# MPI-SWS/RedQueen

Measured on AMD Instinct MI355X. Metric: redqueen_replicas_per_sec, higher is better.
Workload: dtype f64; 1 GPU; C3 syn1k: 1000 followers, 50 sources (25 Poisson2 rate 1 + 25 Hawkes l0=1 a=1 b=10), degree 5, T=100, q=1e6, s=1, RedQueen, randomized worlds; replicas_per_gpu=10000, global_batch=10000, parallelism=replica-sharded dp1, replicas_per_chunk=10000

## Files before the change

redqueen_amd/csrc/rq_api.cpp:

```cpp
#include <hip/hip_runtime.h>

#include <algorithm>
#include <cstring>
#include <memory>
#include <mutex>
#include <new>
#include <vector>

#include "../../include/rq.h"
#include "rq_internal.h"

using rqh::align_up;
using rqh::CtrlTables;
using rqh::GraphTopo;
using rqh::Knobs;
using rqh::Plan;

namespace {

template <class T>
struct DevBuf {
    T* p = nullptr;
    size_t n = 0;
    ~DevBuf() { if (p) (void)hipFree(p); }
// ... 102 lines not shown
        lru->caller = caller;
        lru->used = ++clock;
        return *lru;
    }
};
thread_local SidePipes t_pipes;

}

namespace {
constexpr int kStages = 4;
struct Stage {
    void* buf = nullptr;
    size_t bytes = 0;
    hipEvent_t done = nullptr;
};
}

struct rq_graph : GraphTopo {
    DevBuf<int64_t> d_sink_ids, d_src_id;
    DevBuf<int> d_csr_col_el, d_lay_ptr, d_lay_end;
    DevBuf<int> d_tile_ptr, d_tile_col;
    DevBuf<uint32_t> d_mask, d_fbits;
    DevBuf<int> d_kind, d_orig, d_arr_off, d_arr_n, d_csr_ptr, d_csr_col, d_outdeg_f, d_fol, d_cbf;
    DevBuf<uint32_t> d_seed;
    DevBuf<double> d_p0, d_p1, d_p2, d_arr_a, d_arr_b;
    int upload();
    std::mutex stage_mu;
    Stage stage[kStages];
    int stage_next = 0;
    ~rq_graph()
    {
        for (Stage& st : stage) {
            if (st.done) {
                (void)hipEventSynchronize(st.done);
                (void)hipEventDestroy(st.done);
            }
            if (st.buf) (void)hipHostFree(st.buf);
        }
    }
};

int rq_graph::upload()
{
    int rc;
    if (nw > 0 && (rc = d_mask.upload(masks))) return rc;
    if ((rc = d_fbits.upload(fbits))) return rc;
    if ((rc = d_src_id.upload(src_id)) || (rc = d_kind.upload(kind)) ||
        (rc = d_orig.upload(orig_idx)) || (rc = d_arr_off.upload(arr_off)) ||
        (rc = d_arr_n.upload(arr_n)) || (rc = d_csr_ptr.upload(csr_ptr)) ||
        (rc = d_csr_col.upload(csr_col)) || (rc = d_outdeg_f.upload(outdeg_f)) ||
        (rc = d_fol.upload(fol)) || (rc = d_seed.upload(seed)) ||
        (rc = d_p0.upload(p0)) || (rc = d_p1.upload(p1)) ||
        (rc = d_p2.upload(p2)) || (rc = d_arr_a.upload(arr_a)) ||
        (rc = d_arr_b.upload(arr_b)) || (rc = d_sink_ids.upload(sink_ids)) ||
        (rc = d_csr_col_el.upload(csr_col_el)) || (rc = d_cbf.upload(cbf)))
        return rc;
    if (multi && ((rc = d_lay_ptr.upload(lay_ptr)) || (rc = d_lay_end.upload(lay_end))))
        return rc;
    if (n_tiles > 0 && ((rc = d_tile_ptr.upload(tile_ptr)) || (rc = d_tile_col.upload(tile_col))))
        return rc;
    return RQ_OK;
}

namespace {

double ws_budget(const rq_batch_desc* b, const Knobs& kn, double fallback)
{
    double bud = b && b->ws_budget > 0 ? (double)b->ws_budget : fallback;
    if (!(bud > 0.0)) {
        size_t fr = 0, tot = 0;
        bud = hipMemGetInfo(&fr, &tot) == hipSuccess ? 0.9 * (double)fr : 200.0 * (1 << 30);
    }
    if (kn.ws_budget_gb.set) bud = std::min(bud, kn.ws_budget_gb.v * (1 << 30));
    return bud;
}

int plan_call(const rq_graph* g, const rq_batch_desc* b, const Knobs& kn, double fallback, Plan* p)
{
// ... 64 lines not shown
        return rc;
    }
    ~Join() { (void)done(); }
};
int fork_streams(int nbuf, Join* join)
{
    if (nbuf <= 1) return RQ_OK;
    if (const int rc = join->sp.get(nbuf - 1, join->pst + 1)) return rc;
    if (hipEventRecord(join->sp.fork, join->pst[0]) != hipSuccess) return RQ_EHIP;
    for (int k = 1; k < nbuf; ++k) {
        if (hipStreamWaitEvent(join->pst[k], join->sp.fork, 0) != hipSuccess) return RQ_EHIP;
        join->n = k + 1;
    }
    return RQ_OK;
}

struct Chunk {
    int64_t c0, C;
    char* ws;
    char* wsb;
};

GenArgs gen_args(const rq_graph* g, const Plan& p, const rq_batch_desc* b, const rq_outputs* out,
                 const Chunk& ch)
{
    GenArgs ga{};
    ga.n_chunk = ch.C;
    ga.chunk0 = ch.c0;
    ga.rep0 = b->replica0;
    ga.n_rep = b->n_rep;
    ga.rep_lo = p.rep_lo;
    ga.rep_cnt = p.rep_cnt;
    ga.rep_idx = b->rep_idx ? (const int64_t*)(ch.ws + p.off_repidx) : nullptr;
    ga.n_str = g->n_str;
    ga.ctrl_idx = g->ctrl_idx;
    ga.ctrl_stream_kind =
        (b->ctrl_kind == RQ_SRC_OPT || b->ctrl_kind == RQ_SRC_OPTPW || b->ctrl_kind == RQ_SRC_NONE)
            ? RQ_SRC_NONE : b->ctrl_kind;
    ga.randomize = b->randomize_world;
    ga.seed_mod = b->seed_mod;
    ga.ctrl_seed = b->ctrl_seed;
    ga.ctrl_seed0 = b->ctrl_seed0;
    ga.world_seed = b->world_seed;
    ga.world_seed0 = b->world_seed0;
    ga.ctrl_rate = b->ctrl_rate;
    ga.kind = g->d_kind.p;
    ga.orig_idx = g->d_orig.p;
    ga.seed = g->d_seed.p;
    ga.p0 = g->d_p0.p;
    ga.p1 = g->d_p1.p;
    ga.p2 = g->d_p2.p;
    ga.arr_off = g->d_arr_off.p;
    ga.arr_n = g->d_arr_n.p;
    ga.arr_a = g->d_arr_a.p;
    ga.arr_b = g->d_arr_b.p;
    ga.st_off = (const int64_t*)(ch.ws + p.off_stoff);
    ga.cap = (const int*)(ch.ws + p.off_cap);
    ga.capsum = p.capsum;
    ga.start = g->start;
    ga.end = g->end;
    ga.streams = (double*)(ch.wsb + p.off_streams);
    ga.slen = (int*)(ch.wsb + p.off_slen);
    ga.slen_stride = p.chunk;
    ga.status = out->status;
    if (b->n_rd > 0) {
        ga.rd_k = (const int*)(ch.ws + p.off_rdk);
        ga.n_rd = b->n_rd;
        ga.rd_times = b->rd_times;
        ga.rd_off = b->rd_off;
    }
    return ga;
}

MergeArgs merge_args(const rq_graph* g, const Plan& p, const rq_outputs* out, const Chunk& ch,
                     const GenArgs& ga, const Knobs& kn)
{
    MergeArgs ma{};
    ma.n_chunk = ch.C;
    ma.chunk0 = ch.c0;
    ma.n_str = g->n_str;
    ma.capsum = p.capsum;
    ma.st_off = ga.st_off;
    ma.streams = ga.streams;
    ma.slen = ga.slen;
    ma.slen_stride = ga.slen_stride;
    ma.end = g->end;
    ma.out_t = (double*)(ch.wsb + p.off_mt);
    ma.out_j = (uint16_t*)(ch.wsb + p.off_mj);
    ma.out_jh = g->n_str > 65535 ? (uint8_t*)(ch.wsb + p.off_mjh) : nullptr;
    ma.out_len = (int*)(ch.wsb + p.off_mlen);
    ma.mrg_stride = p.mrg_stride;
    ma.status = out->status;
    ma.strict_ties = p.lmrg ? 1 : 0;
// ... 263 lines not shown
                 size_t workspace_bytes, void* hip_stream)
{
    const Knobs kn = rqh::read_knobs();
    Plan p;
    int rc = plan_call(g, b, kn, (double)workspace_bytes, &p);
    if (rc) return rc;
    if (!out || !out->metrics || !out->counts || !out->status || !workspace) return RQ_EINVAL;
    if (workspace_bytes < p.total) return RQ_EINVAL;
    if ((b->flags & RQ_RUN_EVENT_LOG) && (!out->ev_t || !out->ev_src || out->ev_cap < 1))
        return RQ_EINVAL;
    char* ws = (char*)workspace;
    hipStream_t pst[3] = {(hipStream_t)hip_stream, nullptr, nullptr};

    if ((rc = stage_tables(g, p, b, rqh::ctrl_tables(*g, b), ws, pst[0]))) return rc;
    if (hipMemsetAsync(out->status, 0, sizeof(int32_t) * p.R, pst[0]) != hipSuccess) return RQ_EHIP;
    Join join{pst, t_pipes.of(pst[0])};
    if ((rc = fork_streams(p.nbuf, &join))) return rc;

    int64_t ci = 0;
    for (int64_t c0 = 0; c0 < p.R; c0 += p.chunk, ++ci) {
        hipStream_t s = pst[ci % p.nbuf];
        const Chunk ch{c0, std::min(p.chunk, p.R - c0), ws,
                       ws + p.off_set0 + (size_t)(ci % p.nbuf) * p.set_stride};
        const GenArgs ga = gen_args(g, p, b, out, ch);
        if (!p.fw || p.fwm) {
            TimedLaunch tl(K_GEN, s);
            if (rq_launch_gen(ga, s) != hipSuccess) return RQ_EHIP;
        }
        if (p.mrg && (rc = launch_merge(p, merge_args(g, p, out, ch, ga, kn), ch, s))) return rc;
        const SweepArgs sa = sweep_args(g, p, b, out, ch, ga, kn);
        if (p.order && rq_launch_order(sa.mrg_len, ch.C, (int*)(ch.wsb + p.off_ord), s) != hipSuccess)
            return RQ_EHIP;
        if (hipMemsetAsync(ch.wsb + p.off_wq, 0, 2 * sizeof(int), s) != hipSuccess) return RQ_EHIP;
        {
            TimedLaunch tl(K_SWEEP, s);
            const SweepInst inst = rqh::sweep_inst(p, b->ctrl_kind);
            const hipError_t e = inst.fused ? rq_launch_sweep_fw(sa, inst, s) : rq_launch_sweep(sa, inst, s);
            if (e != hipSuccess) return RQ_EHIP;
        }
        if (p.scan) continue;
        const ScanArgs sc = scan_args(g, p, out, ch, sa);
        TimedLaunch tl(K_SCAN, s);
        if (rq_launch_scan(sc, p.nK, s) != hipSuccess) return RQ_EHIP;
    }
    return join.done();
}

// ... 707 lines not shown
```

redqueen_amd/csrc/rq_gen.h:

```cpp
#pragma once
#include "rq_device.h"
#include "rq_internal.h"

namespace rq {

struct SrcGen {
    uint32_t k0, k1;
    uint32_t d;
    double en, e1n, u2n;
    int kind;
    bool done;
    double t;
    double tau, eta, B;
    double inv;
    double p0, p1, nbeta;
    const uint64_t* etab;
    const double* ta;
    const double* tb;
    int na, ri;

    __device__ __forceinline__ void none()
    {
        etab = nullptr;
        kind = RQ_SRC_NONE;
        done = true;
        d = 0u;
        en = e1n = u2n = 0.0;
    }
    __device__ __forceinline__ void draw2(uint32_t call, double& e, double& u) const
    {
        uint32_t c[4] = {call, 0u, 0u, 0u};
        philox4x32_10(c, k0, k1);
        e = rq_std_exponential(rq_uniform53(c[0], c[1]));
        u = rq_uniform53(c[2], c[3]);
    }

    __device__ __forceinline__ void init(const GenArgs& a, int j, int64_t i, const uint64_t* etab_)
    {
        etab = etab_;
        const bool is_ctrl = j == a.ctrl_idx;
        kind = is_ctrl ? a.ctrl_stream_kind : a.kind[j];
        const int64_t k = a.seed_mod > 0 ? i % a.seed_mod : i;
        uint32_t seed;
        if (is_ctrl) {
            seed = a.ctrl_seed ? a.ctrl_seed[i] : a.ctrl_seed0 + (uint32_t)k;
        } else if (a.randomize) {
            const uint32_t u = a.world_seed ? a.world_seed[i] : a.world_seed0 + (uint32_t)k;
            seed = u + 99u * (uint32_t)a.orig_idx[j];
        } else {
            seed = a.seed[j];
        }
        k0 = seed;
        k1 = kind_salt(kind, is_ctrl);
        d = 0u;
        en = e1n = u2n = 0.0;
        done = false;
        t = a.start;
        tau = a.start;
        eta = 0.0;
        B = 0.0;
        inv = 0.0;
        p0 = p1 = nbeta = 0.0;
        ta = tb = nullptr;
        na = ri = 0;
        if (kind == RQ_SRC_POISSON || kind == RQ_SRC_POISSON2) {
            const double rate = is_ctrl ? a.ctrl_rate[i] : a.p0[j];
            if (rate > 0.0) inv = 1.0 / rate;
            else done = true;
        } else if (kind == RQ_SRC_HAWKES) {
            p0 = a.p0[j];
            p1 = a.p1[j];
            nbeta = -a.p2[j];
            B = p0;
            if (B > 0.0) inv = 1.0 / B;
            else done = true;
        } else if (kind == RQ_SRC_PWCONST) {
            na = a.arr_n[j];
            ta = a.arr_a + a.arr_off[j];
            tb = a.arr_b + a.arr_off[j];
            double mx = tb[0];
            for (int q = 1; q < na; ++q) mx = tb[q] > mx ? tb[q] : mx;
            if (mx > 0.0) inv = 1.0 / mx;
            else done = true;
            p0 = mx;
        } else if (kind == RQ_SRC_REALDATA) {
            const int rk = (a.rd_k && !is_ctrl) ? a.rd_k[j] : -1;
            if (rk >= 0) {
                const int64_t o = a.rd_off[i * a.n_rd + rk];
                na = (int)(a.rd_off[i * a.n_rd + rk + 1] - o);
                ta = a.rd_times + o;
            } else {
                na = a.arr_n[j];
                ta = a.arr_a + a.arr_off[j];
            }
            done = na <= 0;
        } else {
            done = true;
        }
        if (!done && (kind == RQ_SRC_HAWKES || kind == RQ_SRC_PWCONST)) draw2(0u, e1n, u2n);
    }

    __device__ __forceinline__ bool step(double* out, double end)
    {
        if (done) return false;
        if (kind == RQ_SRC_REALDATA) {
            *out = ta[ri];
            ++ri;
            done = ri >= na;
            return true;
        }
        const bool poisson = kind == RQ_SRC_POISSON || kind == RQ_SRC_POISSON2;
        double e, u2 = 0.0;
        if (poisson) {
            if ((d & 1u) == 0u) {
                uint32_t c[4] = {d >> 1, 0u, 0u, 0u};
                philox4x32_10(c, k0, k1);
                e = rq_std_exponential(rq_uniform53(c[0], c[1]));
                en = rq_std_exponential(rq_uniform53(c[2], c[3]));
            } else {
                e = en;
            }
            d += 1u;
        } else {
            e = e1n;
            u2 = u2n;
            d += 2u;
            draw2(d >> 1, e1n, u2n);
        }
        const double tc = t + e * inv;
        if (!(tc <= end)) {
            done = true;
            return false;
        }
        t = tc;
        if (poisson) {
            *out = tc;
            return true;
        }
        if (kind == RQ_SRC_HAWKES) {
            const double decay = rq_exp_t(nbeta * (tc - tau), etab);
            const double rate = p0 + eta * decay;
            const bool acc = u2 * B < rate;
            if (acc) {
                eta = eta * decay + p1;
                tau = tc;
                B = p0 + eta;
            } else {
                B = rate;
            }
            if (B > 0.0) inv = 1.0 / B;
            else done = true;
            if (acc) *out = tc;
            return acc;
        }
        int lo = 0, hi = na;
        while (lo < hi) {
            const int mid = (lo + hi) >> 1;
            if (tc < ta[mid]) hi = mid;
            else lo = mid + 1;
        }
        int idx = lo - 1;
        if (idx < 0) idx += na;
        if (u2 * p0 < tb[idx]) {
            *out = tc;
            return true;
        }
        return false;
    }
};

}
```

redqueen_amd/csrc/rq_host.h:

```cpp
#pragma once
#include <stddef.h>
#include <stdint.h>

#include <vector>

#include "../../include/rq.h"

#define RQ_MAX_STREAMS 2048
#define RQ_NPSUM1_LDS 516
#ifndef RQ_MRG_LB
#define RQ_MRG_LB 1024
#endif
#define RQ_MG_B 512
#define RQ_MAX_STREAMS_MRG (RQ_MG_B * RQ_MG_B)

struct SweepInst {
    bool fused;
    int nK;
    bool col16;
    bool log;
    bool gs;
    bool bits;
    bool bl;
    bool mrg;
// ... 28 lines not shown

inline int followers_tiles(int n_sinks) { return (n_sinks + RQ_FOLLOWERS_TILE_SINKS - 1) / RQ_FOLLOWERS_TILE_SINKS; }
inline size_t followers_tiled_ws_bytes(int n_sinks, int64_t n_rep)
{
    return align_up((size_t)4 * (size_t)n_rep * (size_t)followers_tiles(n_sinks), 256);
}

template <class T>
struct Knob {
    bool set = false;
    T v{};
};
struct Knobs {
    Knob<double> ws_budget_gb;
    double cap_squeeze = 1.0;
    Knob<int> mg_grp;
    bool mrg = true;
    Knob<int> g_collds;
    int g_w = 0;
    bool skip = true;
    bool fwm = true;
    bool ctrl_draws = true;
    bool sweep_scan = true;
    bool phasec_blk = true;
    int fw_w = 0;
    int pipe = 2;
    Knob<int64_t> pipe_chunk;
    bool order = false;

    int sweep_dbg = 0;
    double fw_tile = 58.0;
    Knob<int> fw_hmin, fw_thr, fw_hfill;
    int fw_static = 0;
    bool clk_merge = false;

    Knob<int> rp_chunk;
    bool rp_small = true;
    bool clk_replay = false;

    int lm_of_slots = 4096;
};
Knobs read_knobs();

struct GraphTopo {
    int n_str = 0, ctrl_idx = -1, n_sinks = 0, n_fol = 0;
    int64_t n_edges = 0, ctrl_src_id = 0;
    double start = 0.0, end = 0.0;
    std::vector<int64_t> src_id;
    std::vector<int> kind, orig_idx, arr_off, arr_n;
    std::vector<int> is_static;
    std::vector<uint32_t> seed;
    std::vector<double> p0, p1, p2, arr_a, arr_b;
    std::vector<int> csr_ptr, csr_col, outdeg_f, fol;
    std::vector<int64_t> fol_ids;
    std::vector<int64_t> sink_ids;
    std::vector<int> csr_col_el;
    std::vector<int> col_to_fol;
    bool multi = false, ctrl_dup = false;
    bool rd_ties = false, rd_ties_ctrl = false;
    std::vector<int> lay_ptr, lay_end;
    int nw = 0;
    std::vector<uint32_t> masks;
    std::vector<uint32_t> fbits;
    std::vector<int> cbf;
    int n_tiles = 0;
    std::vector<int> tile_ptr, tile_col;
    int ctrl_arr_off = 0, ctrl_arr_n = 0;
};
int topo_build(const rq_graph_desc* d, GraphTopo* g);

struct Plan {
    int nK = 1, spl = 1, wpb = 4, n_sinks_pad = 0;
    int64_t R = 0, chunk = 0, capsum = 0, cap_rows = 0;
    int64_t rep_lo = 0, rep_cnt = 0;
    std::vector<int> cap;
    std::vector<int64_t> st_off;
    std::vector<int> rd_k;
    bool log = false, bits = false;
    bool bl = false;
    size_t g_fb = 0, g_etab = 0, g_inv = 0, g_skip = 0;
    bool g_inv_sh = false;
    bool gs = false;
    int64_t gs_slots = 0, gs_stride = 0;
    bool fw = false;
    int fw_h = 8, mstride = 1;
    bool mrg = false;
    bool lmrg = false;
// ... 68 lines not shown
```

redqueen_amd/csrc/rq_internal.h:

```cpp
#pragma once
#include <hip/hip_runtime.h>
#include <stdint.h>

#include <map>
#include <mutex>
#include <tuple>

#include "../../include/rq.h"
#include "rq_host.h"
#include "rq_log_walk.h"

__host__ __device__ __forceinline__ int64_t rq_global_replica(int64_t s, int64_t n_rep, int64_t rep_lo,
                                                               int64_t rep_cnt)
{
    return rep_cnt == n_rep ? s : (s / rep_cnt) * n_rep + rep_lo + s % rep_cnt;
}

struct GenArgs {
    int64_t n_chunk, chunk0, rep0;
    int64_t n_rep, rep_lo, rep_cnt;
    const int64_t* rep_idx;
    int n_str, ctrl_idx, ctrl_stream_kind, randomize;
    int64_t seed_mod;
    const uint32_t* ctrl_seed;
    uint32_t ctrl_seed0;
    const uint32_t* world_seed;
    uint32_t world_seed0;
    const double* ctrl_rate;
    const int* kind;
    const int* orig_idx;
    const uint32_t* seed;
    const double *p0, *p1, *p2;
    const int *arr_off, *arr_n;
    const double *arr_a, *arr_b;
    const int64_t* st_off;
    const int* cap;
    int64_t capsum;
    double start, end;
    double* streams;
    int* slen;
    int64_t slen_stride;
    int32_t* status;
    const int* rd_k;
    int n_rd;
    const double* rd_times;
    const int64_t* rd_off;
};

__host__ __device__ __forceinline__ int64_t rq_replica_of(const GenArgs& a, int64_t local)
{
    return a.rep_idx ? a.rep_idx[local] : rq_global_replica(a.rep0 + local, a.n_rep, a.rep_lo, a.rep_cnt);
}

struct SweepArgs {
    int64_t n_chunk, chunk0, n_rep, rep0;
    int wpb, n_str, n_sinks, n_sinks_pad, ctrl_idx, ctrl_kind, n_fol;
    int Ks[RQ_MAX_K];
    int64_t ctrl_src_id;
    int64_t seed_mod;
    const uint32_t* ctrl_seed;
    uint32_t ctrl_seed0;
    const int64_t* src_id;
    const double* inv_c;
    const double* pw_c;
    const double* pw_max;
    int n_seg;
    double period;
    const int* csr_ptr;
    const int* csr_col;
// ... 387 lines not shown
```

redqueen_amd/csrc/rq_kernels.hip:

```cpp
#include <hip/hip_runtime.h>
#include <stdint.h>

#include "rq_device.h"
#include "rq_internal.h"
#include "rq_sweep_core.h"
#include "rq_gen.h"
#include "rq_scan_rows.h"
#include <type_traits>
#include <algorithm>
#include <cstdlib>

#pragma clang fp contract(off)

using namespace rq;

__global__ __launch_bounds__(256) void rq_gen_streams(GenArgs a)
{
    __shared__ uint64_t etab[RQ_EXP_TAB_N];
    for (int e = threadIdx.x; e < RQ_EXP_TAB_N; e += blockDim.x) etab[e] = rq_exp_tab_c[e];
    __syncthreads();
    const int64_t rl = (int64_t)blockIdx.x * blockDim.x + threadIdx.x;
    const int j = (int)(blockIdx.z * gridDim.y + blockIdx.y);
    if (rl >= a.n_chunk || j >= a.n_str) return;
    const int64_t o = a.chunk0 + rl;
    const int64_t i = rq_replica_of(a, o);
    SrcGen gen;
    gen.init(a, j, i, etab);

    double* out = a.streams + rl * a.capsum + a.st_off[j];
    const int cap = a.cap[j];
    int n = 0;
    bool ovf = false;
#ifndef RQ_GEN_W
#define RQ_GEN_W 16
#endif
    constexpr int GW = RQ_GEN_W;
    static_assert(GW == 8 || GW == 16, "staging width");
    double sb[GW];
#pragma unroll
    for (int k = 0; k < GW; ++k) sb[k] = 0.0;
    while (!gen.done && !ovf) {
        double tv;
        if (gen.step(&tv, a.end)) {
            if (n < cap) {
#pragma unroll
                for (int k = 0; k + 1 < GW; ++k) sb[k] = sb[k + 1];
                sb[GW - 1] = tv;
                ++n;
                if ((n & (GW - 1)) == 0) {
                    double4* d = reinterpret_cast<double4*>(out + n - GW);
#pragma unroll
                    for (int k = 0; k < GW / 4; ++k) d[k] = make_double4(sb[4 * k], sb[4 * k + 1], sb[4 * k + 2], sb[4 * k + 3]);
                }
            } else {
                ovf = true;
            }
        }
    }
    {
        const int r = n & (GW - 1);
        if (r > 0) {
#ifndef RQ_GEN_TAIL_STEPS
#define RQ_GEN_TAIL_STEPS 1
#endif
            const int sh = GW - r;
#pragma unroll
            for (int st = 1; st < GW; st <<= 1) {
                const bool on = (sh & st) != 0;
#pragma unroll
                for (int k = 0; k < GW; ++k) {
#if RQ_GEN_TAIL_STEPS
                    const double up = sb[k + st < GW ? k + st : GW - 1], keep = sb[k];
                    sb[k] = on ? up : keep;
#else
                    sb[k] = on ? sb[k + st < GW ? k + st : GW - 1] : sb[k];
#endif
                }
            }
            double4* d = reinterpret_cast<double4*>(out + (n - r));
#pragma unroll
            for (int k = 0; k < GW / 4; ++k)
                if (k < 2 || r > 8) d[k] = make_double4(sb[4 * k], sb[4 * k + 1], sb[4 * k + 2], sb[4 * k + 3]);
        }
    }
    a.slen[(int64_t)j * a.slen_stride + rl] = n;
    if (ovf) atomicOr(&a.status[o], RQ_ST_STREAM_OVERFLOW);
}

template <int SPL, int NK, class COL, int W, bool LOG, bool BITS, bool BL, bool GS = false, bool MRG = false,
          bool GT = false>
__global__ __launch_bounds__(LOG ? 256 : (MRG ? RQ_MRG_LB : (SPL >= 4 ? 512 : 1024))) void rq_sweep(SweepArgs a)
{
    extern __shared__ double lds_g[];
    char* base = reinterpret_cast<char*>(lds_g);
    const int lane = lane_id();
    const int w = __builtin_amdgcn_readfirstlane((int)(threadIdx.x >> 6));
    int* cptr = reinterpret_cast<int*>(base + a.lds_ptr);
    int* odf = reinterpret_cast<int*>(base + a.lds_odf);
    int* cbf = reinterpret_cast<int*>(base + a.lds_cbf);
    constexpr bool col_lds = sizeof(COL) == 2;
    COL* col_l = reinterpret_cast<COL*>(base + a.lds_col);
    const int* col_g = a.csr_col;
    if (col_lds && !BITS)
        for (int e = threadIdx.x; e < a.n_csr; e += blockDim.x) col_l[e] = (COL)a.csr_col[e];
    uint32_t* msk = reinterpret_cast<uint32_t*>(base + a.lds_mask);
    if (BITS)
        for (int e = threadIdx.x; e < a.n_str * a.mstride; e += blockDim.x) {
            const int jj = e / a.mstride, ww = e - jj * a.mstride;
            msk[e] = ww < a.nw ? a.masks[jj * a.nw + ww] : 0u;
        }
// ... 908 lines not shown
}

static int occ_t(SweepKernel k, int wpb, size_t lds)
{
    return rq_occupancy(k, 64 * wpb, lds);
}
static hipError_t launch_sweep_t(SweepKernel k, bool gs, const SweepArgs& a, hipStream_t s)
{
    unsigned blocks = (unsigned)((a.n_chunk + a.wpb - 1) / a.wpb);
    if (a.wq) {
        const int nb_c = occ_t(k, a.wpb, a.lds_total);
        const unsigned cap = (unsigned)(nb_c > 0 ? nb_c : 1) * (unsigned)rq_cu_count();
        if (cap < blocks) blocks = cap;
    }
    if (gs) {
        const unsigned cap = (unsigned)(a.gs_slots / a.wpb);
        if (!a.wq || cap < 1) return hipErrorInvalidValue;
        if (cap < blocks) blocks = cap;
    }
    hipLaunchKernelGGL(k, dim3(blocks), dim3(64 * a.wpb), a.lds_total, s, a);
    return hipGetLastError();
}

hipError_t rq_launch_gen(const GenArgs& a, hipStream_t s)
{
    if (a.n_chunk <= 0 || a.n_str <= 0) return hipSuccess;
    const unsigned gy = (unsigned)std::min(a.n_str, 32768);
    dim3 grid((unsigned)((a.n_chunk + 255) / 256), gy, (unsigned)((a.n_str + gy - 1) / gy));
    hipLaunchKernelGGL(rq_gen_streams, grid, dim3(256), 0, s, a);
    return hipGetLastError();
}

hipError_t rq_launch_sweep(const SweepArgs& a, const SweepInst& i, hipStream_t s)
{
    if (a.n_chunk <= 0) return hipSuccess;
    const SweepKernel k = sweep_kernel(i);
    return k ? launch_sweep_t(k, i.log && i.gs, a, s) : hipErrorInvalidValue;
}

int rq_sweep_blocks_per_cu(const SweepInst& i, int wpb, size_t lds)
{
    const SweepKernel k = sweep_kernel(i);
    return k ? occ_t(k, wpb, lds) : 0;
}

template <int NK>
static hipError_t launch_scan_t(const ScanArgs& a, hipStream_t s)
{
    const size_t lds = 4 * npsum_lds_doubles<NK + 2>() * sizeof(double);
    constexpr auto k = rq_scan<NK, 2>;
    unsigned blocks = (unsigned)((a.n_chunk + 3) / 4);
    if (a.wq) {
        const int nb = rq_occupancy(k, 256, lds);
        const unsigned cap = (unsigned)(nb > 0 ? nb : 1) * (unsigned)rq_cu_count();
        if (cap < blocks) blocks = cap;
// ... 16 lines not shown
```

redqueen_amd/csrc/rq_plan.cpp:

```cpp
#include <algorithm>
#include <cmath>
#include <cstdlib>

#include "rq_host.h"
#include "rq_tables.h"

namespace rqh {

Knobs read_knobs()
{
    Knobs k;
    if (const char* e = getenv("RQ_WS_BUDGET_GB")) k.ws_budget_gb = {true, atof(e)};
    if (const char* e = getenv("RQ_CAP_SQUEEZE")) k.cap_squeeze = std::max(0.01, std::min(1.0, atof(e)));
    if (const char* e = getenv("RQ_MG_GRP")) k.mg_grp = {true, atoi(e)};
    if (const char* e = getenv("RQ_MRG")) k.mrg = atoi(e) != 0;
    if (const char* e = getenv("RQ_G_COLLDS")) k.g_collds = {true, atoi(e)};
    if (const char* e = getenv("RQ_G_W")) k.g_w = atoi(e);
    if (const char* e = getenv("RQ_SKIP")) k.skip = atoi(e) != 0;
    if (const char* e = getenv("RQ_FWM")) k.fwm = atoi(e) != 0;
    if (const char* e = getenv("RQ_CTRL_DRAWS")) k.ctrl_draws = atoi(e) != 0;
    if (const char* e = getenv("RQ_SWEEP_SCAN")) k.sweep_scan = atoi(e) != 0;
    if (const char* e = getenv("RQ_PHASEC_BLK")) k.phasec_blk = atoi(e) != 0;
    if (const char* e = getenv("RQ_FW_W")) k.fw_w = atoi(e);
    if (const char* e = getenv("RQ_PIPE")) k.pipe = std::max(1, std::min(3, atoi(e)));
    if (const char* e = getenv("RQ_PIPE_CHUNK")) k.pipe_chunk = {true, std::max<int64_t>(64, atoll(e))};
    if (const char* e = getenv("RQ_ORDER")) k.order = atoi(e) != 0;
    if (const char* e = getenv("RQ_SWEEP_DBG")) k.sweep_dbg = atoi(e);
    if (const char* e = getenv("RQ_FW_TILE")) k.fw_tile = atof(e);
    if (const char* e = getenv("RQ_FW_HMIN")) k.fw_hmin = {true, atoi(e)};
    if (const char* e = getenv("RQ_FW_THR")) k.fw_thr = {true, atoi(e)};
    if (const char* e = getenv("RQ_FW_HFILL")) k.fw_hfill = {true, atoi(e)};
    static const int fw_static = getenv("RQ_FW_STATIC") ? atoi(getenv("RQ_FW_STATIC")) : 0;
    k.fw_static = fw_static;
    k.clk_merge = getenv("RQ_CLK_MERGE") != nullptr;
    if (const char* e = getenv("RQ_RP_CHUNK")) k.rp_chunk = {true, atoi(e)};
    if (const char* e = getenv("RQ_RP_SMALL")) k.rp_small = atoi(e) != 0;
    k.clk_replay = getenv("RQ_CLK_REPLAY") != nullptr;
    if (const char* e = getenv("RQ_LM_OF_SLOTS")) k.lm_of_slots = std::max(1, std::min(4096, atoi(e)));
    return k;
}

namespace {

constexpr size_t kLdsMax = 160 * 1024;
// ... 484 lines not shown
```

redqueen_amd/csrc/rq_spec.h:

```cpp
#ifndef RQ_SPEC_H
#define RQ_SPEC_H

#include <stdint.h>
#include <math.h>
#include "rq_tables.h"

#if defined(__HIPCC__)
#define RQ_HD __host__ __device__ __forceinline__
#define RQ_HD_COLD static __host__ __device__ __attribute__((noinline))
#pragma clang fp contract(off)
#else
#define RQ_HD static inline
#define RQ_HD_COLD static
#endif

RQ_HD uint64_t rq_dbl_bits(double x)
{
    union { double d; uint64_t u; } c;
    c.d = x;
    return c.u;
}

RQ_HD double rq_bits_dbl(uint64_t u)
{
    union { double d; uint64_t u; } c;
    c.u = u;
    return c.d;
}

RQ_HD double rq_uniform53(uint32_t a, uint32_t b)
{
    return ((double)(a >> 5) * 67108864.0 + (double)(b >> 6)) / 9007199254740992.0;
}

RQ_HD double rq_log(double x)
{
    const double ln2_hi = 6.93147180369123816490e-01;
    const double ln2_lo = 1.90821492927058770002e-10;
    const double Lg1 = 6.666666666666735130e-01;
    const double Lg2 = 3.999999999940941908e-01;
    const double Lg3 = 2.857142874366239149e-01;
    const double Lg4 = 2.222219843214978396e-01;
    const double Lg5 = 1.818357216161805012e-01;
    const double Lg6 = 1.531383769920937332e-01;
    const double Lg7 = 1.479819860511658591e-01;

    uint64_t ux = rq_dbl_bits(x);
    if (!(x > 0.0)) {
        if (x == 0.0) return rq_bits_dbl(0xfff0000000000000ull);
        return rq_bits_dbl(0x7ff8000000000000ull);
    }
    if ((ux >> 52) >= 0x7ffu) return x + x;

    int32_t k = 0;
    if ((ux >> 52) == 0) {
        x = x * 18014398509481984.0;
        ux = rq_dbl_bits(x);
        k = -54;
    }
    int32_t hx = (int32_t)(ux >> 32);
    k += (hx >> 20) - 1023;
    hx &= 0x000fffff;
    int32_t i = (hx + 0x95f64) & 0x100000;
    uint64_t um = ((uint64_t)(uint32_t)(hx | (i ^ 0x3ff00000)) << 32) | (ux & 0xffffffffu);
    k += (i >> 20);
    double f = rq_bits_dbl(um) - 1.0;
    double dk = (double)k;

    double s = f / (2.0 + f);
    double z = s * s;
    double w = z * z;
    double t1 = w * (Lg2 + w * (Lg4 + w * Lg6));
    double t2 = z * (Lg1 + w * (Lg3 + w * (Lg5 + w * Lg7)));
    double R = t2 + t1;
    double hfsq = 0.5 * f * f;
    if (f == 0.0) return dk * ln2_hi + dk * ln2_lo;
    return dk * ln2_hi - ((hfsq - (s * (hfsq + R) + dk * ln2_lo)) - f);
}

RQ_HD double rq_exp_core(double x, const uint64_t* tab, uint64_t adj)
{
    const double kd0 = x * RQ_EXP_INVLN2N + 0x1.8p52;
    const uint64_t ki = rq_dbl_bits(kd0);
    const double kd = kd0 - 0x1.8p52;
    double r = fma(kd, -RQ_EXP_LN2HI, x);
    r = fma(kd, -RQ_EXP_LN2LO, r);
    const uint32_t j = (uint32_t)ki & 31u;
    const double tail = rq_bits_dbl(tab[2 * j]);
    const double sc = rq_bits_dbl(tab[2 * j + 1] + (ki << 47) + adj);
    const double r2 = r * r;
    const double c6 = rq_bits_dbl(tab[64]), c24 = rq_bits_dbl(tab[65]);
    const double c120 = rq_bits_dbl(tab[66]), c720 = rq_bits_dbl(tab[67]);
    const double p = fma(r, fma(r, fma(r, fma(r, c720, c120), c24), c6), 0.5);
    const double tmp = fma(r2, p, r) + tail;
    return fma(sc, tmp, sc);
}

RQ_HD_COLD double rq_exp_special(double x, const uint64_t* tab)
{
    if (x != x) return x + x;
// ... 23 lines not shown
```

redqueen_amd/csrc/rq_topo.cpp:

```cpp
#include <algorithm>
#include <cmath>
#include <unordered_map>
#include <vector>

#include "rq_host.h"

namespace rqh {

namespace {
constexpr int kBitsMaxSinks = 2048;
}

int topo_build(const rq_graph_desc* d, GraphTopo* g)
{
    if (!d || !g) return RQ_EINVAL;
    if (d->n_sinks < 1 || !d->sink_ids) return RQ_EINVAL;
    if (d->n_sources < 0 || (d->n_sources > 0 && !d->sources)) return RQ_EINVAL;
    if (d->n_edges < 0 || (d->n_edges > 0 && (!d->edge_src || !d->edge_sink))) return RQ_EINVAL;
    if (!(d->end_time >= d->start_time)) return RQ_EINVAL;
    g->start = d->start_time;
    g->end = d->end_time;
    g->ctrl_src_id = d->ctrl_src_id;

    std::vector<int64_t> sinks(d->sink_ids, d->sink_ids + d->n_sinks);
// ... 144 lines not shown
        }
        if (layers.empty()) g->lay_end.push_back((int)g->csr_col.size());
        g->lay_ptr.push_back((int)g->lay_end.size());
        g->outdeg_f.push_back(of);
        g->csr_ptr.push_back((int)g->csr_col.size());
        for (int c : rows[j]) g->csr_col_el.push_back(c);
    }

    if (g->n_sinks <= kBitsMaxSinks) {
        g->nw = (g->n_sinks + 31) / 32;
        g->masks.assign((size_t)g->n_str * g->nw, 0u);
        for (int j = 0; j < g->n_str; ++j)
            for (int e = g->csr_ptr[j]; e < g->csr_ptr[j + 1]; ++e) {
                const int c = g->csr_col[e];
                g->masks[(size_t)j * g->nw + c / 32] |= 1u << (c % 32);
            }
    }

    g->fbits.assign((g->n_sinks + 31) / 32, 0u);
    for (int c : g->fol) g->fbits[c / 32] |= 1u << (c % 32);
    g->cbf.resize(g->n_str);
    for (int j = 0; j < g->n_str; ++j) g->cbf[j] = g->is_static[j] || g->ctrl_src_id < g->src_id[j];

    if (!g->multi && g->n_sinks <= RQ_FOLLOWERS_TILED_MAX_SINKS) {
        const int TS = RQ_FOLLOWERS_TILE_SINKS;
        const int nt = followers_tiles(g->n_sinks);
        const size_t stride = (size_t)g->n_str + 1;
        g->n_tiles = nt;
        g->tile_ptr.assign((size_t)nt * stride, 0);
        g->tile_col.resize(g->csr_col_el.size());
        std::vector<int> at((size_t)nt * g->n_str, 0);
        for (int j = 0; j < g->n_str; ++j)
            for (int e = g->csr_ptr[j]; e < g->csr_ptr[j + 1]; ++e)
                ++at[(size_t)(g->csr_col_el[e] / TS) * g->n_str + j];
        int off = 0;
        for (int i = 0; i < nt; ++i) {
            for (int j = 0; j < g->n_str; ++j) {
                g->tile_ptr[i * stride + j] = off;
                const int n = at[(size_t)i * g->n_str + j];
                at[(size_t)i * g->n_str + j] = off;
                off += n;
            }
            g->tile_ptr[i * stride + g->n_str] = off;
        }
        for (int j = 0; j < g->n_str; ++j)
            for (int e = g->csr_ptr[j]; e < g->csr_ptr[j + 1]; ++e) {
// ... 134 lines not shown
```

Measured before the change: 4.724 million replicas/s.

## Split stream generation by source class with specialized Poisson and Hawkes kernels

Streams are grouped on the host into Hawkes, Poisson and other classes, and the generation kernel dispatches each block row to a class-specialized path. Hawkes rows use a kind-templated generator with the branches resolved at compile time. Poisson rows use a batched generator that draws 16 exponentials per iteration and writes them with vector stores. A straight-line log skips special-case checks on the uniform draw. The aim is to remove warp divergence and per-step kind branching in the generator, at the cost of extra code paths and a log variant whose results must stay bitwise-identical.

After: 4.968 million replicas/s (median of 6 runs). 1.05x the previous value.

```diff
diff --git a/redqueen_amd/csrc/rq_api.cpp b/redqueen_amd/csrc/rq_api.cpp
--- a/redqueen_amd/csrc/rq_api.cpp
+++ b/redqueen_amd/csrc/rq_api.cpp
@@ -148,7 +148,7 @@
     DevBuf<int> d_csr_col_el, d_lay_ptr, d_lay_end;
     DevBuf<int> d_tile_ptr, d_tile_col;
     DevBuf<uint32_t> d_mask, d_fbits;
-    DevBuf<int> d_kind, d_orig, d_arr_off, d_arr_n, d_csr_ptr, d_csr_col, d_outdeg_f, d_fol, d_cbf;
+    DevBuf<int> d_kind, d_orig, d_arr_off, d_arr_n, d_csr_ptr, d_csr_col, d_outdeg_f, d_fol, d_cbf, d_gen_cls;
     DevBuf<uint32_t> d_seed;
     DevBuf<double> d_p0, d_p1, d_p2, d_arr_a, d_arr_b;
     int upload();
@@ -180,7 +180,8 @@
         (rc = d_p0.upload(p0)) || (rc = d_p1.upload(p1)) ||
         (rc = d_p2.upload(p2)) || (rc = d_arr_a.upload(arr_a)) ||
         (rc = d_arr_b.upload(arr_b)) || (rc = d_sink_ids.upload(sink_ids)) ||
-        (rc = d_csr_col_el.upload(csr_col_el)) || (rc = d_cbf.upload(cbf)))
+        (rc = d_csr_col_el.upload(csr_col_el)) || (rc = d_cbf.upload(cbf)) ||
+        (rc = d_gen_cls.upload(gen_cls)))
         return rc;
     if (multi && ((rc = d_lay_ptr.upload(lay_ptr)) || (rc = d_lay_end.upload(lay_end))))
         return rc;
@@ -291,7 +292,7 @@
 };
 
 GenArgs gen_args(const rq_graph* g, const Plan& p, const rq_batch_desc* b, const rq_outputs* out,
-                 const Chunk& ch)
+                 const Chunk& ch, const Knobs& kn)
 {
     GenArgs ga{};
     ga.n_chunk = ch.C;
@@ -338,6 +339,10 @@
         ga.rd_times = b->rd_times;
         ga.rd_off = b->rd_off;
     }
+    if (kn.gen_split) {
+        ga.cls = g->d_gen_cls.p;
+        for (int c = 0; c < 3; ++c) ga.cls_n[c] = g->gen_n[c];
+    }
     return ga;
 }
 
@@ -647,7 +652,7 @@
         hipStream_t s = pst[ci % p.nbuf];
         const Chunk ch{c0, std::min(p.chunk, p.R - c0), ws,
                        ws + p.off_set0 + (size_t)(ci % p.nbuf) * p.set_stride};
-        const GenArgs ga = gen_args(g, p, b, out, ch);
+        const GenArgs ga = gen_args(g, p, b, out, ch, kn);
         if (!p.fw || p.fwm) {
             TimedLaunch tl(K_GEN, s);
             if (rq_launch_gen(ga, s) != hipSuccess) return RQ_EHIP;
diff --git a/redqueen_amd/csrc/rq_gen.h b/redqueen_amd/csrc/rq_gen.h
--- a/redqueen_amd/csrc/rq_gen.h
+++ b/redqueen_amd/csrc/rq_gen.h
@@ -4,7 +4,24 @@
 
 namespace rq {
 
-struct SrcGen {
+__device__ __forceinline__ uint32_t gen_seed(const GenArgs& a, int j, int64_t i, bool is_ctrl)
+{
+    const int64_t k = a.seed_mod > 0 ? i % a.seed_mod : i;
+    if (is_ctrl) return a.ctrl_seed ? a.ctrl_seed[i] : a.ctrl_seed0 + (uint32_t)k;
+    if (a.randomize) {
+        const uint32_t u = a.world_seed ? a.world_seed[i] : a.world_seed0 + (uint32_t)k;
+        return u + 99u * (uint32_t)a.orig_idx[j];
+    }
+    return a.seed[j];
+}
+
+__device__ __forceinline__ double gen_exponential(uint32_t w0, uint32_t w1)
+{
+    return -rq_log_normal(rq_dbl_bits(1.0 - rq_uniform53(w0, w1)), 0, 1);
+}
+
+template <int KIND = -1>
+struct SrcGenT {
     uint32_t k0, k1;
     uint32_t d;
     double en, e1n, u2n;
@@ -19,6 +36,8 @@
     const double* tb;
     int na, ri;
 
+    __device__ __forceinline__ bool is(int k) const { return KIND < 0 ? kind == k : KIND == k; }
+
     __device__ __forceinline__ void none()
     {
         etab = nullptr;
@@ -31,7 +50,7 @@
     {
         uint32_t c[4] = {call, 0u, 0u, 0u};
         philox4x32_10(c, k0, k1);
-        e = rq_std_exponential(rq_uniform53(c[0], c[1]));
+        e = KIND < 0 ? rq_std_exponential(rq_uniform53(c[0], c[1])) : gen_exponential(c[0], c[1]);
         u = rq_uniform53(c[2], c[3]);
     }
 
@@ -40,17 +59,7 @@
         etab = etab_;
         const bool is_ctrl = j == a.ctrl_idx;
         kind = is_ctrl ? a.ctrl_stream_kind : a.kind[j];
-        const int64_t k = a.seed_mod > 0 ? i % a.seed_mod : i;
-        uint32_t seed;
-        if (is_ctrl) {
-            seed = a.ctrl_seed ? a.ctrl_seed[i] : a.ctrl_seed0 + (uint32_t)k;
-        } else if (a.randomize) {
-            const uint32_t u = a.world_seed ? a.world_seed[i] : a.world_seed0 + (uint32_t)k;
-            seed = u + 99u * (uint32_t)a.orig_idx[j];
-        } else {
-            seed = a.seed[j];
-        }
-        k0 = seed;
+        k0 = gen_seed(a, j, i, is_ctrl);
         k1 = kind_salt(kind, is_ctrl);
         d = 0u;
         en = e1n = u2n = 0.0;
@@ -63,18 +72,18 @@
         p0 = p1 = nbeta = 0.0;
         ta = tb = nullptr;
         na = ri = 0;
-        if (kind == RQ_SRC_POISSON || kind == RQ_SRC_POISSON2) {
+        if (is(RQ_SRC_POISSON) || is(RQ_SRC_POISSON2)) {
             const double rate = is_ctrl ? a.ctrl_rate[i] : a.p0[j];
             if (rate > 0.0) inv = 1.0 / rate;
             else done = true;
-        } else if (kind == RQ_SRC_HAWKES) {
+        } else if (is(RQ_SRC_HAWKES)) {
             p0 = a.p0[j];
             p1 = a.p1[j];
             nbeta = -a.p2[j];
             B = p0;
             if (B > 0.0) inv = 1.0 / B;
             else done = true;
-        } else if (kind == RQ_SRC_PWCONST) {
+        } else if (is(RQ_SRC_PWCONST)) {
             na = a.arr_n[j];
             ta = a.arr_a + a.arr_off[j];
             tb = a.arr_b + a.arr_off[j];
@@ -83,7 +92,7 @@
             if (mx > 0.0) inv = 1.0 / mx;
             else done = true;
             p0 = mx;
-        } else if (kind == RQ_SRC_REALDATA) {
+        } else if (is(RQ_SRC_REALDATA)) {
             const int rk = (a.rd_k && !is_ctrl) ? a.rd_k[j] : -1;
             if (rk >= 0) {
                 const int64_t o = a.rd_off[i * a.n_rd + rk];
@@ -97,19 +106,19 @@
         } else {
             done = true;
         }
-        if (!done && (kind == RQ_SRC_HAWKES || kind == RQ_SRC_PWCONST)) draw2(0u, e1n, u2n);
+        if (!done && (is(RQ_SRC_HAWKES) || is(RQ_SRC_PWCONST))) draw2(0u, e1n, u2n);
     }
 
     __device__ __forceinline__ bool step(double* out, double end)
     {
         if (done) return false;
-        if (kind == RQ_SRC_REALDATA) {
+        if (is(RQ_SRC_REALDATA)) {
             *out = ta[ri];
             ++ri;
             done = ri >= na;
             return true;
         }
-        const bool poisson = kind == RQ_SRC_POISSON || kind == RQ_SRC_POISSON2;
+        const bool poisson = is(RQ_SRC_POISSON) || is(RQ_SRC_POISSON2);
         double e, u2 = 0.0;
         if (poisson) {
             if ((d & 1u) == 0u) {
@@ -137,7 +146,7 @@
             *out = tc;
             return true;
         }
-        if (kind == RQ_SRC_HAWKES) {
+        if (is(RQ_SRC_HAWKES)) {
             const double decay = rq_exp_t(nbeta * (tc - tau), etab);
             const double rate = p0 + eta * decay;
             const bool acc = u2 * B < rate;
@@ -168,5 +177,6 @@
         return false;
     }
 };
+using SrcGen = SrcGenT<>;
 
 }
diff --git a/redqueen_amd/csrc/rq_gen.hip b/redqueen_amd/csrc/rq_gen.hip
--- /dev/null
+++ b/redqueen_amd/csrc/rq_gen.hip
@@ -0,0 +1,202 @@
+#include <hip/hip_runtime.h>
+#include <stdint.h>
+
+#include "rq_device.h"
+#include "rq_internal.h"
+#include "rq_gen.h"
+#include <algorithm>
+
+#pragma clang fp contract(off)
+
+using namespace rq;
+
+namespace {
+
+struct GenRows {
+    int l0, ln, rows;
+};
+__device__ __forceinline__ int gen_row() { return (int)(blockIdx.z * gridDim.y + blockIdx.y); }
+__device__ __forceinline__ int gen_stream(const GenArgs& a, const GenRows& g, int r)
+{
+    return a.cls ? (r < g.ln ? a.cls[g.l0 + r] : a.ctrl_idx) : r;
+}
+
+__device__ __forceinline__ void gen_load_etab(uint64_t* etab)
+{
+    for (int e = threadIdx.x; e < RQ_EXP_TAB_N; e += blockDim.x) etab[e] = rq_exp_tab_c[e];
+    __syncthreads();
+}
+
+template <int KIND>
+__device__ __forceinline__ void gen_steps(const GenArgs& a, int j, int64_t rl, const uint64_t* etab)
+{
+    const int64_t o = a.chunk0 + rl;
+    const int64_t i = rq_replica_of(a, o);
+    SrcGenT<KIND> gen;
+    gen.init(a, j, i, etab);
+
+    double* out = a.streams + rl * a.capsum + a.st_off[j];
+    const int cap = a.cap[j];
+    int n = 0;
+    bool ovf = false;
+#ifndef RQ_GEN_W
+#define RQ_GEN_W 16
+#endif
+    constexpr int GW = RQ_GEN_W;
+    static_assert(GW == 8 || GW == 16, "staging width");
+    double sb[GW];
+#pragma unroll
+    for (int k = 0; k < GW; ++k) sb[k] = 0.0;
+    while (!gen.done && !ovf) {
+        double tv;
+        if (gen.step(&tv, a.end)) {
+            if (n < cap) {
+#pragma unroll
+                for (int k = 0; k + 1 < GW; ++k) sb[k] = sb[k + 1];
+                sb[GW - 1] = tv;
+                ++n;
+                if ((n & (GW - 1)) == 0) {
+                    double4* d = reinterpret_cast<double4*>(out + n - GW);
+#pragma unroll
+                    for (int k = 0; k < GW / 4; ++k) d[k] = make_double4(sb[4 * k], sb[4 * k + 1], sb[4 * k + 2], sb[4 * k + 3]);
+                }
+            } else {
+                ovf = true;
+            }
+        }
+    }
+    {
+        const int r = n & (GW - 1);
+        if (r > 0) {
+#ifndef RQ_GEN_TAIL_STEPS
+#define RQ_GEN_TAIL_STEPS 1
+#endif
+            const int sh = GW - r;
+#pragma unroll
+            for (int st = 1; st < GW; st <<= 1) {
+                const bool on = (sh & st) != 0;
+#pragma unroll
+                for (int k = 0; k < GW; ++k) {
+#if RQ_GEN_TAIL_STEPS
+                    const double up = sb[k + st < GW ? k + st : GW - 1], keep = sb[k];
+                    sb[k] = on ? up : keep;
+#else
+                    sb[k] = on ? sb[k + st < GW ? k + st : GW - 1] : sb[k];
+#endif
+                }
+            }
+            double4* d = reinterpret_cast<double4*>(out + (n - r));
+#pragma unroll
+            for (int k = 0; k < GW / 4; ++k)
+                if (k < 2 || r > 8) d[k] = make_double4(sb[4 * k], sb[4 * k + 1], sb[4 * k + 2], sb[4 * k + 3]);
+        }
+    }
+    a.slen[(int64_t)j * a.slen_stride + rl] = n;
+    if (ovf) atomicOr(&a.status[o], RQ_ST_STREAM_OVERFLOW);
+}
+
+__device__ __forceinline__ void gen_poisson(const GenArgs& a, int j, int64_t rl)
+{
+    const int64_t o = a.chunk0 + rl;
+    const int64_t i = rq_replica_of(a, o);
+    const bool is_ctrl = j == a.ctrl_idx;
+    const uint32_t k0 = gen_seed(a, j, i, is_ctrl);
+    const uint32_t k1 = kind_salt(is_ctrl ? a.ctrl_stream_kind : a.kind[j], is_ctrl);
+    const double rate = is_ctrl ? a.ctrl_rate[i] : a.p0[j];
+    const double end = a.end;
+    double* out = a.streams + rl * a.capsum + a.st_off[j];
+    const int cap = a.cap[j];
+    bool done = !(rate > 0.0), ovf = false;
+    const double inv = done ? 0.0 : 1.0 / rate;
+    double t = a.start;
+    int n = 0;
+    while (!done) {
+        if (n >= cap) {
+            uint32_t c[4] = {(uint32_t)n >> 1, 0u, 0u, 0u};
+            philox4x32_10(c, k0, k1);
+            const double tc = t + gen_exponential(c[0], c[1]) * inv;
+            ovf = tc <= end;
+            break;
+        }
+        double sb[16];
+        int m = 0;
+        bool ok = true;
+        double tc = t;
+#pragma unroll
+        for (int q = 0; q < 16; q += 2) {
+            uint32_t c[4] = {((uint32_t)n + q) >> 1, 0u, 0u, 0u};
+            philox4x32_10(c, k0, k1);
+            const double e[2] = {gen_exponential(c[0], c[1]), gen_exponential(c[2], c[3])};
+#pragma unroll
+            for (int h = 0; h < 2; ++h) {
+                tc = tc + e[h] * inv;
+                ok = ok && tc <= end;
+                m += ok ? 1 : 0;
+                sb[q + h] = tc;
+            }
+        }
+        double4* d = reinterpret_cast<double4*>(out + n);
+#pragma unroll
+        for (int k = 0; k < 4; ++k)
+            if (k < 2 ? m > 0 : m > 8) d[k] = make_double4(sb[4 * k], sb[4 * k + 1], sb[4 * k + 2], sb[4 * k + 3]);
+        n += m;
+        t = sb[15];
+        done = m < 16;
+    }
+    a.slen[(int64_t)j * a.slen_stride + rl] = n;
+    if (ovf) atomicOr(&a.status[o], RQ_ST_STREAM_OVERFLOW);
+}
+
+}
+
+__global__ __launch_bounds__(256) void rq_gen_streams(GenArgs a, GenRows g)
+{
+    __shared__ uint64_t etab[RQ_EXP_TAB_N];
+    gen_load_etab(etab);
+    const int64_t rl = (int64_t)blockIdx.x * blockDim.x + threadIdx.x;
+    const int r = gen_row();
+    if (rl >= a.n_chunk || r >= g.rows) return;
+    gen_steps<-1>(a, gen_stream(a, g, r), rl, etab);
+}
+
+__global__ __launch_bounds__(256) void rq_gen_classes(GenArgs a, GenRows h, GenRows p, GenRows g)
+{
+    __shared__ uint64_t etab[RQ_EXP_TAB_N];
+    const int64_t rl = (int64_t)blockIdx.x * blockDim.x + threadIdx.x;
+    int r = gen_row();
+    if (r >= h.rows + p.rows + g.rows) return;
+    if (r < h.rows) {
+        gen_load_etab(etab);
+        if (rl < a.n_chunk) gen_steps<RQ_SRC_HAWKES>(a, gen_stream(a, h, r), rl, etab);
+    } else if ((r -= h.rows) < p.rows) {
+        if (rl < a.n_chunk) gen_poisson(a, gen_stream(a, p, r), rl);
+    } else {
+        gen_load_etab(etab);
+        if (rl < a.n_chunk) gen_steps<-1>(a, gen_stream(a, g, r - p.rows), rl, etab);
+    }
+}
+
+namespace {
+template <class K, class... R>
+void launch_rows(K k, const GenArgs& a, int rows, hipStream_t s, R... r)
+{
+    const unsigned gy = (unsigned)std::min(rows, 32768);
+    dim3 grid((unsigned)((a.n_chunk + 255) / 256), gy, ((unsigned)rows + gy - 1) / gy);
+    hipLaunchKernelGGL(k, grid, dim3(256), 0, s, a, r...);
+}
+}
+
+hipError_t rq_launch_gen(const GenArgs& a, hipStream_t s)
+{
+    if (a.n_chunk <= 0 || a.n_str <= 0) return hipSuccess;
+    if (!a.cls) {
+        launch_rows(rq_gen_streams, a, a.n_str, s, GenRows{0, a.n_str, a.n_str});
+        return hipGetLastError();
+    }
+    const int ck = a.ctrl_stream_kind;
+    const int cc = ck == RQ_SRC_HAWKES ? 0 : (ck == RQ_SRC_POISSON || ck == RQ_SRC_POISSON2) ? 1 : 2;
+    GenRows c[3];
+    for (int k = 0, l0 = 0; k < 3; l0 += a.cls_n[k], ++k) c[k] = GenRows{l0, a.cls_n[k], a.cls_n[k] + (k == cc ? 1 : 0)};
+    launch_rows(rq_gen_classes, a, a.n_str, s, c[0], c[1], c[2]);
+    return hipGetLastError();
+}
diff --git a/redqueen_amd/csrc/rq_host.h b/redqueen_amd/csrc/rq_host.h
--- a/redqueen_amd/csrc/rq_host.h
+++ b/redqueen_amd/csrc/rq_host.h
@@ -74,6 +74,7 @@
     bool fwm = true;
     bool ctrl_draws = true;
     bool sweep_scan = true;
+    bool gen_split = true;
     bool phasec_blk = true;
     int fw_w = 0;
     int pipe = 2;
@@ -115,6 +116,8 @@
     std::vector<uint32_t> masks;
     std::vector<uint32_t> fbits;
     std::vector<int> cbf;
+    std::vector<int> gen_cls;
+    int gen_n[3] = {0, 0, 0};
     int n_tiles = 0;
     std::vector<int> tile_ptr, tile_col;
     int ctrl_arr_off = 0, ctrl_arr_n = 0;
diff --git a/redqueen_amd/csrc/rq_internal.h b/redqueen_amd/csrc/rq_internal.h
--- a/redqueen_amd/csrc/rq_internal.h
+++ b/redqueen_amd/csrc/rq_internal.h
@@ -45,6 +45,8 @@
     int n_rd;
     const double* rd_times;
     const int64_t* rd_off;
+    const int* cls;
+    int cls_n[3];
 };
 
 __host__ __device__ __forceinline__ int64_t rq_replica_of(const GenArgs& a, int64_t local)
diff --git a/redqueen_amd/csrc/rq_kernels.hip b/redqueen_amd/csrc/rq_kernels.hip
--- a/redqueen_amd/csrc/rq_kernels.hip
+++ b/redqueen_amd/csrc/rq_kernels.hip
@@ -14,78 +14,6 @@
 
 using namespace rq;
 
-__global__ __launch_bounds__(256) void rq_gen_streams(GenArgs a)
-{
-    __shared__ uint64_t etab[RQ_EXP_TAB_N];
-    for (int e = threadIdx.x; e < RQ_EXP_TAB_N; e += blockDim.x) etab[e] = rq_exp_tab_c[e];
-    __syncthreads();
-    const int64_t rl = (int64_t)blockIdx.x * blockDim.x + threadIdx.x;
-    const int j = (int)(blockIdx.z * gridDim.y + blockIdx.y);
-    if (rl >= a.n_chunk || j >= a.n_str) return;
-    const int64_t o = a.chunk0 + rl;
-    const int64_t i = rq_replica_of(a, o);
-    SrcGen gen;
-    gen.init(a, j, i, etab);
-
-    double* out = a.streams + rl * a.capsum + a.st_off[j];
-    const int cap = a.cap[j];
-    int n = 0;
-    bool ovf = false;
-#ifndef RQ_GEN_W
-#define RQ_GEN_W 16
-#endif
-    constexpr int GW = RQ_GEN_W;
-    static_assert(GW == 8 || GW == 16, "staging width");
-    double sb[GW];
-#pragma unroll
-    for (int k = 0; k < GW; ++k) sb[k] = 0.0;
-    while (!gen.done && !ovf) {
-        double tv;
-        if (gen.step(&tv, a.end)) {
-            if (n < cap) {
-#pragma unroll
-                for (int k = 0; k + 1 < GW; ++k) sb[k] = sb[k + 1];
-                sb[GW - 1] = tv;
-                ++n;
-                if ((n & (GW - 1)) == 0) {
-                    double4* d = reinterpret_cast<double4*>(out + n - GW);
-#pragma unroll
-                    for (int k = 0; k < GW / 4; ++k) d[k] = make_double4(sb[4 * k], sb[4 * k + 1], sb[4 * k + 2], sb[4 * k + 3]);
-                }
-            } else {
-                ovf = true;
-            }
-        }
-    }
-    {
-        const int r = n & (GW - 1);
-        if (r > 0) {
-#ifndef RQ_GEN_TAIL_STEPS
-#define RQ_GEN_TAIL_STEPS 1
-#endif
-            const int sh = GW - r;
-#pragma unroll
-            for (int st = 1; st < GW; st <<= 1) {
-                const bool on = (sh & st) != 0;
-#pragma unroll
-                for (int k = 0; k < GW; ++k) {
-#if RQ_GEN_TAIL_STEPS
-                    const double up = sb[k + st < GW ? k + st : GW - 1], keep = sb[k];
-                    sb[k] = on ? up : keep;
-#else
-                    sb[k] = on ? sb[k + st < GW ? k + st : GW - 1] : sb[k];
-#endif
-                }
-            }
-            double4* d = reinterpret_cast<double4*>(out + (n - r));
-#pragma unroll
-            for (int k = 0; k < GW / 4; ++k)
-                if (k < 2 || r > 8) d[k] = make_double4(sb[4 * k], sb[4 * k + 1], sb[4 * k + 2], sb[4 * k + 3]);
-        }
-    }
-    a.slen[(int64_t)j * a.slen_stride + rl] = n;
-    if (ovf) atomicOr(&a.status[o], RQ_ST_STREAM_OVERFLOW);
-}
 
 template <int SPL, int NK, class COL, int W, bool LOG, bool BITS, bool BL, bool GS = false, bool MRG = false,
           bool GT = false>
@@ -1040,15 +968,6 @@
     return hipGetLastError();
 }
 
-hipError_t rq_launch_gen(const GenArgs& a, hipStream_t s)
-{
-    if (a.n_chunk <= 0 || a.n_str <= 0) return hipSuccess;
-    const unsigned gy = (unsigned)std::min(a.n_str, 32768);
-    dim3 grid((unsigned)((a.n_chunk + 255) / 256), gy, (unsigned)((a.n_str + gy - 1) / gy));
-    hipLaunchKernelGGL(rq_gen_streams, grid, dim3(256), 0, s, a);
-    return hipGetLastError();
-}
-
 hipError_t rq_launch_sweep(const SweepArgs& a, const SweepInst& i, hipStream_t s)
 {
     if (a.n_chunk <= 0) return hipSuccess;
diff --git a/redqueen_amd/csrc/rq_plan.cpp b/redqueen_amd/csrc/rq_plan.cpp
--- a/redqueen_amd/csrc/rq_plan.cpp
+++ b/redqueen_amd/csrc/rq_plan.cpp
@@ -20,6 +20,7 @@
     if (const char* e = getenv("RQ_FWM")) k.fwm = atoi(e) != 0;
     if (const char* e = getenv("RQ_CTRL_DRAWS")) k.ctrl_draws = atoi(e) != 0;
     if (const char* e = getenv("RQ_SWEEP_SCAN")) k.sweep_scan = atoi(e) != 0;
+    if (const char* e = getenv("RQ_GEN_SPLIT")) k.gen_split = atoi(e) != 0;
     if (const char* e = getenv("RQ_PHASEC_BLK")) k.phasec_blk = atoi(e) != 0;
     if (const char* e = getenv("RQ_FW_W")) k.fw_w = atoi(e);
     if (const char* e = getenv("RQ_PIPE")) k.pipe = std::max(1, std::min(3, atoi(e)));
diff --git a/redqueen_amd/csrc/rq_spec.h b/redqueen_amd/csrc/rq_spec.h
--- a/redqueen_amd/csrc/rq_spec.h
+++ b/redqueen_amd/csrc/rq_spec.h
@@ -33,7 +33,7 @@
     return ((double)(a >> 5) * 67108864.0 + (double)(b >> 6)) / 9007199254740992.0;
 }
 
-RQ_HD double rq_log(double x)
+RQ_HD double rq_log_normal(uint64_t ux, int32_t k, int straight)
 {
     const double ln2_hi = 6.93147180369123816490e-01;
     const double ln2_lo = 1.90821492927058770002e-10;
@@ -45,19 +45,6 @@
     const double Lg6 = 1.531383769920937332e-01;
     const double Lg7 = 1.479819860511658591e-01;
 
-    uint64_t ux = rq_dbl_bits(x);
-    if (!(x > 0.0)) {
-        if (x == 0.0) return rq_bits_dbl(0xfff0000000000000ull);
-        return rq_bits_dbl(0x7ff8000000000000ull);
-    }
-    if ((ux >> 52) >= 0x7ffu) return x + x;
-
-    int32_t k = 0;
-    if ((ux >> 52) == 0) {
-        x = x * 18014398509481984.0;
-        ux = rq_dbl_bits(x);
-        k = -54;
-    }
     int32_t hx = (int32_t)(ux >> 32);
     k += (hx >> 20) - 1023;
     hx &= 0x000fffff;
@@ -74,8 +61,26 @@
     double t2 = z * (Lg1 + w * (Lg3 + w * (Lg5 + w * Lg7)));
     double R = t2 + t1;
     double hfsq = 0.5 * f * f;
-    if (f == 0.0) return dk * ln2_hi + dk * ln2_lo;
+    if (!straight && f == 0.0) return dk * ln2_hi + dk * ln2_lo;
     return dk * ln2_hi - ((hfsq - (s * (hfsq + R) + dk * ln2_lo)) - f);
+}
+
+RQ_HD double rq_log(double x)
+{
+    uint64_t ux = rq_dbl_bits(x);
+    if (!(x > 0.0)) {
+        if (x == 0.0) return rq_bits_dbl(0xfff0000000000000ull);
+        return rq_bits_dbl(0x7ff8000000000000ull);
+    }
+    if ((ux >> 52) >= 0x7ffu) return x + x;
+
+    int32_t k = 0;
+    if ((ux >> 52) == 0) {
+        x = x * 18014398509481984.0;
+        ux = rq_dbl_bits(x);
+        k = -54;
+    }
+    return rq_log_normal(ux, k, 0);
 }
 
 RQ_HD double rq_exp_core(double x, const uint64_t* tab, uint64_t adj)
diff --git a/redqueen_amd/csrc/rq_topo.cpp b/redqueen_amd/csrc/rq_topo.cpp
--- a/redqueen_amd/csrc/rq_topo.cpp
+++ b/redqueen_amd/csrc/rq_topo.cpp
@@ -190,6 +190,19 @@
     g->cbf.resize(g->n_str);
     for (int j = 0; j < g->n_str; ++j) g->cbf[j] = g->is_static[j] || g->ctrl_src_id < g->src_id[j];
 
+    g->gen_cls.clear();
+    for (int c = 0; c < 3; ++c) {
+        g->gen_n[c] = 0;
+        for (int j = 0; j < g->n_str; ++j) {
+            if (j == g->ctrl_idx) continue;
+            const int k = g->kind[j];
+            const int cj = k == RQ_SRC_HAWKES ? 0 : (k == RQ_SRC_POISSON || k == RQ_SRC_POISSON2) ? 1 : 2;
+            if (cj != c) continue;
+            g->gen_cls.push_back(j);
+            ++g->gen_n[c];
+        }
+    }
+
     if (!g->multi && g->n_sinks <= RQ_FOLLOWERS_TILED_MAX_SINKS) {
         const int TS = RQ_FOLLOWERS_TILE_SINKS;
         const int nt = followers_tiles(g->n_sinks);
```
